# inhavl-shlee/AFI-GAN

Measured on AMD Instinct MI355X. Metric: stage1_G+D_step_images_per_s, higher is better.
Workload: dtype f32 via f16x3: two scaled fp16 pieces per operand, three f16 MFMAs per product, fp32 accumulate (tensors fp32)

## Files before the change

### afigan_amd/csrc/afi_common.h

```cpp
#pragma once
#include <hip/hip_runtime.h>
#include <stdint.h>
#include "../../include/afigan_hip.h"

typedef float f32x16 __attribute__((ext_vector_type(16)));
typedef float f32x4 __attribute__((ext_vector_type(4)));

#define AFI_LRELU_SLOPE 0.2f

#ifndef AFI_TRY
#define AFI_TRY(expr) do { int _s = (expr); if (_s != AFI_OK) return _s; } while (0)
#endif

struct AfiView {
    float* p;
    long long sN, sH, sW;
};

struct AfiBnLoad { const float* mean; const float* invstd; const float* gamma; const float* beta; };

struct AfiPixGemm {
    int N, H, W;
    int ntaps;
    int Ck;
// ... 38 lines not shown
#define AFI_WK6_STAGE_BYTES 6144
struct AfiWk6ImgJob { const float* B; long long b_sRow, b_sTap; int Ncols, Ck, ntaps, nKphase, b_rc; unsigned char* dst; };
struct AfiWk6Side { float* zero_p; long long zero_n4; const float* bl_dout; float* bl_dx; int bl_N, bl_H, bl_W, bl_C; };
struct AfiWk6ConvT { const float* W; unsigned char* dst; float* pack_dst; int Cin, Cout, mode, pad_; };

struct AfiWgradGemm {
    int N, H, W;
    int ntaps;
    int Mrows;
    int Ncols;
    AfiView DY; int dy_up; int CoutPhase;
    AfiView X;
    int x_stride, xH, xW;
    float* DW; long long dw_sRow, dw_sTap;
    long long dy_sTap, x_sTap;
    float alpha;
    int splitK;
};

#ifndef AFI_WINO4_POINTS
#define AFI_WINO4_POINTS 1
#endif
struct AfiF16Bound { const float* amax; int stride; int pad_; float cmul[36]; };

struct AfiColsumProb { const float* g; float* db; long long P, ld; int C; float alpha; };

static inline int afi_cdiv(long long a, long long b) { return (int)((a + b - 1) / b); }
```

### afigan_amd/csrc/afi_f16_split.h

```cpp
#pragma once
#include "afi_common.h"
typedef float f32x2 __attribute__((ext_vector_type(2)));
typedef unsigned int u32x2 __attribute__((ext_vector_type(2)));
typedef unsigned int u32x4 __attribute__((ext_vector_type(4)));
typedef _Float16 f16x8 __attribute__((ext_vector_type(8)));
typedef _Float16 f16x2 __attribute__((ext_vector_type(2)));


__device__ __forceinline__ float afi_f16_scale(float bound) {
    unsigned e = (__float_as_uint(bound) >> 23) & 0xffu;
    e = e < 27u ? 27u : e;
    return __uint_as_float((268u - e) << 23);
}
__device__ __forceinline__ float afi_pow2_inverse(float s) { return __uint_as_float((254u << 23) - __float_as_uint(s)); }

__device__ __forceinline__ void afi_split2_f16_pair(float x0, float x1, float s, unsigned& hi, unsigned& lo) {
    unsigned h, l;
    asm("v_fma_mixlo_f16 %0, %1, %2, 0" : "=v"(h) : "v"(x0), "v"(s));
    asm("v_fma_mixhi_f16 %0, %1, %2, 0" : "+v"(h) : "v"(x1), "v"(s));
    asm("v_fma_mixlo_f16 %0, %1, %2, -%3 op_sel:[0,0,0] op_sel_hi:[0,0,1]" : "=v"(l) : "v"(x0), "v"(s), "v"(h));
    asm("v_fma_mixhi_f16 %0, %1, %2, -%3 op_sel:[0,0,1] op_sel_hi:[0,0,1]" : "+v"(l) : "v"(x1), "v"(s), "v"(h));
    hi = h; lo = l;
}
__device__ __forceinline__ void afi_split2_f16_pair_cvt(float x0, float x1, float s, unsigned& hi, unsigned& lo) {
    const float a = x0 * s, b = x1 * s;
    const f16x2 h = __builtin_convertvector((f32x2){a, b}, f16x2);
    hi = __builtin_bit_cast(unsigned, h);
    const float r0 = a - (float)h[0], r1 = b - (float)h[1];
    lo = __builtin_bit_cast(unsigned, __builtin_convertvector((f32x2){r0, r1}, f16x2));
}
__device__ __forceinline__ void afi_split2_f16_x8_cvt(f32x4 v0, f32x4 v1, float s, u32x4& h, u32x4& l) {
    unsigned h0, h1, h2, h3, l0, l1, l2, l3;
    afi_split2_f16_pair_cvt(v0[0], v0[1], s, h0, l0);
    afi_split2_f16_pair_cvt(v0[2], v0[3], s, h1, l1);
    afi_split2_f16_pair_cvt(v1[0], v1[1], s, h2, l2);
    afi_split2_f16_pair_cvt(v1[2], v1[3], s, h3, l3);
    h = u32x4{h0, h1, h2, h3};
// ... 12 lines not shown
```

### afigan_amd/csrc/afi_launch.h

```cpp
#pragma once
#include "afi_common.h"

int afi_launch_pix_gemm(const AfiPixGemm& p, int b_rc, hipStream_t st);
int afi_launch_gemm_tn(const float* Q, const float* V, float* dU, int planes, long long rows_per_plane, int M, int N, hipStream_t st, bool deterministic = false);
int afi_launch_gemm_nt(const float* A, const float* B, float* C, int planes, long long rows_per_plane, int N, int K, hipStream_t st);
int afi_launch_split_bf16_tiles(const float* B, void* out, int planes, int N, int K, int split, hipStream_t st);
int afi_launch_gemm_nt_bf16_dma(const float* A, const void* Bsplit, float* C, int planes, long long rows_per_plane, int N, int K, int split, hipStream_t st);
int afi_launch_gemm_tn_bf16(const float* Q, const float* V, float* dU, int planes, long long rows_per_plane, int M, int N, int split, hipStream_t st, bool deterministic = false);
int afi_launch_split_f16_tiles(const float* B, void* out, int planes, int N, int K, hipStream_t st, int wkind = 0);
int afi_f16_image_begin(void* out, hipStream_t st);
float* afi_f16_image_wmax(void* out);
long long afi_f16_image_bytes(int planes, int N, int K);
int afi_launch_absmax_planes(const float* X, long long per_plane, int planes, float* out, hipStream_t st);
AfiF16Bound afi_f16_bound(const float* amax, int kind);
int afi_launch_gemm_nt_f16x3(const float* A, const void* Bimg, float* C, int planes, long long rows_per_plane, int N, int K, const AfiF16Bound& ab, hipStream_t st,
                             bool a_pre = false, long long nt256_min_tiles = 512, bool local_sums = false);
int afi_launch_gemm_tn_f16x3(const float* Q, const float* V, float* dU, int planes, long long rows_per_plane, int M, int N, const AfiF16Bound& qb, const AfiF16Bound& vb,
                             hipStream_t st, bool pre = false, bool deterministic = false);
int afi_launch_wgrad_gemm(const AfiWgradGemm& p, hipStream_t st);
int afi_launch_wgrad_gemm_group(const AfiWgradGemm* probs, int n, int wide, hipStream_t st);
int afi_launch_wgrad_gemm_group6(const AfiWgradGemm* probs, int n, hipStream_t st);
int afi_launch_pix_gemm_group(const AfiPixGemm* probs, int n, int b_rc, hipStream_t st);

long long afi_wk6_image_bytes(int Ncols, int Ck, int ntaps, int nKphase);
// ... 50 lines not shown
int afi_launch_maxpool3s2_same(AfiView x, int N, int H, int W, int C, float* out, hipStream_t st);
int afi_launch_fuse_swish(const float* a, const float* b, const float* c, const float* w, float* out, long long n, hipStream_t st);
int afi_launch_sgd(const void* descs_dev, int ntensors, long long max_n, float lr, float mom, float gscale, hipStream_t st);
int afi_launch_scale(float* p, long long n, float s, hipStream_t st);
int afi_launch_sum_accum(const float* v, long long n, float alpha, float* out, hipStream_t st);
int afi_launch_inc_i64(long long* p, hipStream_t st);
int afi_launch_invstd(const float* var, float* invstd, int C, hipStream_t st);

#ifndef AFI_STATS_MAX_ROWS
#define AFI_STATS_MAX_ROWS 1024
#endif
int afi_wino_stats_rows(long long T, int C);
int afi_launch_wino_weight(const float* w, float* U, int O, int I, int mode, hipStream_t st, float* wmax = nullptr);
int afi_launch_wino_input(AfiView x, int N, int H, int W, int C, long long Tpad, float* V, hipStream_t st, long long ldo = 0, float* amax = nullptr,
                          const AfiF16Bound* pre = nullptr);
int afi_launch_wino_output(const float* M, long long Tpad, int N, int H, int W, int C, const float* bias, float alpha, AfiView out, AfiView z,
                           hipStream_t st);
int afi_launch_wino_output_epi(const float* M, long long Tpad, const AfiPixGemm& p, hipStream_t st);
int afi_launch_wino_dy(AfiView dy, int N, int H, int W, int C, long long Tpad, float* Q, hipStream_t st, long long ldo = 0, float* amax = nullptr, const AfiF16Bound* pre = nullptr);
int afi_launch_wino_dw(const float* dU, float* dW, int O, int I, float alpha, hipStream_t st);
int afi_launch_wino4_input(AfiView x, int N, int H, int W, int C, long long Tpad, float* V, hipStream_t st, long long ldo = 0, float* amax = nullptr,
                           const AfiF16Bound* pre = nullptr);
int afi_launch_wino4_weight(const float* w, float* U, int O, int I, int mode, hipStream_t st, float* wmax = nullptr);
int afi_launch_wino4_output_epi(const float* M, long long Tpad, const AfiPixGemm& p, hipStream_t st);
int afi_launch_wino4_dy(AfiView dy, int N, int H, int W, int C, long long Tpad, float* Q, hipStream_t st, long long ldo = 0, float* amax = nullptr, const AfiF16Bound* pre = nullptr);
int afi_launch_wino4_dw(const float* dU, float* dW, int O, int I, float alpha, hipStream_t st);
```

### afigan_amd/csrc/nets.hip

```cpp
#include <string.h>
#include <stdlib.h>

#include "../../include/afigan_hip.h"
#include "afi_common.h"
#include "afi_launch.h"
#include <initializer_list>
#include <new>


#include <vector>
namespace {
struct SideStream {
    hipStream_t side = nullptr;
    std::vector<hipEvent_t> ring;
    size_t next = 0;
    bool init() {
        if (side) return true;
        if (hipStreamCreateWithFlags(&side, hipStreamNonBlocking) != hipSuccess) { side = nullptr; return false; }
        ring.resize(128);
        for (auto& e : ring)
            if (hipEventCreateWithFlags(&e, hipEventDisableTiming) != hipSuccess) return false;
        return true;
    }
    void destroy() {
// ... 181 lines not shown
static bool wino_eligible(const afi_ctx* cx, const AfiPixGemm& g, int b_rc) {
    if (!afi_opt(cx, AFI_OPT_WINOGRAD) || g.ntaps != 9 || g.gtap || g.r2_post) return false;
    const bool phases = g.nKphase == 4 && g.a_up == 2 && b_rc;
    if (!phases && (g.nKphase != 1 || g.a_up != 1)) return false;
    if (g.Ck < 128 || g.Ncols < 128 || (g.Ck & 3) || (g.Ncols & 3)) return false;
    if ((long long)g.N * g.H * g.W < wino_g_minpix(cx)) return false;
    const int I = b_rc ? g.Ncols : g.Ck;
    return g.b_sTap == I && g.b_sRow == 9LL * I && g.a_sgn == (b_rc ? -1 : 1);
}
static float* wino_wcache_slot(afi_ctx* cx, const float* w, int f4, int mode, int O, int I, long long need, bool& hit) {
    hit = false;
    if (!cx || !cx->wcache.buf) return nullptr;
    WinoWeightCache& c = cx->wcache;
    for (int i = 0; i < c.n; ++i) {
        const WinoWeightCache::Entry& e = c.e[i];
        if (e.w == w && e.f4 == f4 && e.mode == mode && e.O == O && e.I == I) { hit = true; return c.buf + e.off; }
    }
    if (c.n == 128 || c.used + need > c.floats) return nullptr;
    c.e[c.n++] = WinoWeightCache::Entry{w, f4, mode, O, I, c.used};
    float* slot = c.buf + c.used;
    c.used += need;
    return slot;
}

constexpr long long kWk6MaxPixels = 8192;
constexpr int kWk6MaxReq = 24;
struct Wk6Req { const float* key; const float* src; int Ncols, Ck, nKphase, b_rc; long long b_sRow, b_sTap; int convT; float* pack_dst; };
static inline Wk6Req wk6_req(const float* key, const float* src, int Ncols, int Ck, int nKphase, int b_rc, long long b_sRow, long long b_sTap) {
    return Wk6Req{key, src, Ncols, Ck, nKphase, b_rc, b_sRow, b_sTap, 0, nullptr};
}
static inline long long wk6_req_floats(int Ncols, int Ck, int nKphase) { return align4((afi_wk6_image_bytes(Ncols, Ck, 9, nKphase) + 3) / 4); }
struct Wk6Images {
    bool on = false;
    int n = 0;
    struct Ent { const float* key; const unsigned char* img; int nstages; } e[kWk6MaxReq];
    void attach(AfiPixGemm& g, const float* key, int c_lo = 0) const {
        if (!on || (c_lo & 31)) return;
        for (int i = 0; i < n; ++i)
            if (e[i].key == key) { g.Bimg = e[i].img; g.bimg_nstages = e[i].nstages; g.bimg_stage0 = (c_lo / 32) * g.ntaps; return; }
    }
};
static int wk6_build(afi_ctx* cx, Wk6Images& im, const Wk6Req* reqs, int n, float* arena, long long arena_floats, hipStream_t st,
                     const AfiWk6Side* side = nullptr, bool* side_done = nullptr, bool* ct_built = nullptr) {
    im.on = false; im.n = 0;
    if (side_done) *side_done = false;
    if (ct_built) *ct_built = false;
    if (n > kWk6MaxReq) return AFI_OK;
    struct CacheRollback {
        afi_ctx* cx; int n0; long long used0; bool keep = false;
        explicit CacheRollback(afi_ctx* c) : cx(c), n0(c ? c->wcache.n : 0), used0(c ? c->wcache.used : 0) {}
        ~CacheRollback() { if (cx && !keep) { cx->wcache.n = n0; cx->wcache.used = used0; } }
    } rollback(cx);
    AfiWk6ImgJob jobs[kWk6MaxReq];
    AfiWk6ConvT ct;
    bool have_ct = false;
    int nj = 0;
    long long used = 0;
    for (int i = 0; i < n; ++i) {
        const Wk6Req& r = reqs[i];
        const long long need = wk6_req_floats(r.Ncols, r.Ck, r.nKphase);
        bool hit = false;
        float* slot = wino_wcache_slot(cx, r.key,  4 + r.b_rc, r.nKphase, r.Ncols, r.Ck, need, hit);
        if (!slot) {
            if (!arena || used + need > arena_floats) { im.n = 0; return AFI_OK; }
            slot = arena + used; used += need; hit = false;
        }
        const int nst = afi_cdiv(r.Ck, 32) * 9 * r.nKphase;
        if (!hit && r.convT) {
            if (have_ct) { im.n = 0; return AFI_OK; }
            ct = AfiWk6ConvT{r.src, (unsigned char*)slot, r.pack_dst, r.convT == 1 ? r.Ck : r.Ncols, r.convT == 1 ? r.Ncols / 4 : r.Ck, r.convT == 1 ? 0 : 1, 0};
            have_ct = true;
        } else if (!hit) {
            jobs[nj++] = AfiWk6ImgJob{r.src, r.b_sRow, r.b_sTap, r.Ncols, r.Ck, 9, r.nKphase, r.b_rc, (unsigned char*)slot};
        }
        im.e[im.n++] = Wk6Images::Ent{r.key, (const unsigned char*)slot, nst};
// ... 3 lines not shown
        if (side && side_done) *side_done = true;
        if (have_ct && ct_built) *ct_built = true;
    }
    rollback.keep = true;
    im.on = true;
    return AFI_OK;
}
static inline bool wk6_shapes_ok(int C, int G, int R) { return (C % 32) == 0 && (G % 32) == 0 && 6 * R + 4 <= kWk6MaxReq; }
constexpr long long kWk6HiResMaxPixels = 4096;
static long long gen_wk6_fwd_floats(int C, int G, int R, long long P) {
    if (P > kWk6MaxPixels || !wk6_shapes_ok(C, G, R)) return 0;
    const int L = C + 4 * G;
    long long f = 3 * wk6_req_floats(C, C, 1) + wk6_req_floats(4 * C, C, 1);
    for (int k = 1; k <= 4; ++k) f += (long long)R * wk6_req_floats(G, C + (k - 1) * G, 1);
    return f + (long long)R * wk6_req_floats(C, L, 1);
}
static long long gen_wk6_bwd_floats(int C, int G, int R, long long P) {
    if (P > kWk6MaxPixels || !wk6_shapes_ok(C, G, R)) return 0;
    const int L = C + 4 * G;
    long long f = 3 * wk6_req_floats(C, C, 1) + wk6_req_floats(C, C, 4);
    for (int k = 1; k <= 4; ++k) f += (long long)R * wk6_req_floats(C + (k - 1) * G, G, 1);
    return f + (long long)R * wk6_req_floats(L, C, 1);
}

static int wino_run(afi_ctx* cx, const AfiPixGemm& g, const WinoForm& f, float* ws, long long ws_floats, float* part, long long part_floats, hipStream_t st) {
    AFI_TRY(afi_o16_refused(g));
    const int b_rc = f.kind == kWinoDgrad;
    const int nph = g.nKphase;
    const int K = g.Ck * nph, Nc = g.Ncols;
    if (ws_floats < wino_ws_floats(g.N, g.H, g.W, K, Nc)) return AFI_ERR_WORKSPACE;
    const int dtype = f.dtype, np = f.np; const long long Tpad = f.Tpad;
    const bool f4 = f.f4, dma = f.dma, f16 = f.f16;
    float* U = ws;
    float* Vb = U + align4((long long)np * K * Nc);
    float* Mb = Vb + align4(np * Tpad * K);
    float* Usp = Mb + align4(np * Tpad * Nc);
    float* amax = nullptr;
    bool have_u = false;
    if (g.no_wcache) {
    } else if (dma) {
        if (float* slot = wino_wcache_slot(cx, g.B, f4, b_rc | (dtype << 4), b_rc ? K : Nc, b_rc ? Nc : K, wino_usplit_floats(np, (long long)K * Nc), have_u)) Usp = slot;
    } else if (float* slot = wino_wcache_slot(cx, g.B, f4, b_rc, b_rc ? K : Nc, b_rc ? Nc : K, align4((long long)np * K * Nc), have_u)) U = slot;
    if (!have_u) {
        float* wmax = dma && f16 ? afi_f16_image_wmax(Usp) : nullptr;
        if (wmax) AFI_TRY(afi_f16_image_begin(Usp, st));
        AFI_TRY(f4 ? afi_launch_wino4_weight(g.B, U, b_rc ? K : Nc, b_rc ? Nc : K, b_rc, st, wmax)
                   : afi_launch_wino_weight(g.B, U, b_rc ? K : Nc, b_rc ? Nc : K, b_rc, st, wmax));
        if (dma) AFI_TRY(f16 ? afi_launch_split_f16_tiles(U, Usp, np, Nc, K, st, f4 ? 6 : 5) : afi_launch_split_bf16_tiles(U, Usp, np, Nc, K, dtype, st));
    }
    const bool a_pre = f.presplit && g.a_amax && g.a_amax_known;
    if (f16 && !(amax = g.a_amax ? g.a_amax : wino_amax_take(cx, ws, ws_floats, 1, st))) return AFI_ERR_LAUNCH;
    const AfiF16Bound abound = afi_f16_bound(amax, f4 ? 2 : 1);
    if (g.v_keep && !(f.keep && a_pre)) return AFI_ERR_BAD_ARG;
    if (g.v_keep) Vb = g.v_keep;
    for (int ph = 0; ph < nph; ++ph) {
        AfiView a = g.A;
        if (nph == 4) { a.p += (ph >> 1) * g.A.sH + (ph & 1) * g.A.sW; a.sH *= 2; a.sW *= 2; }
        float* raise = g.a_amax ? (g.a_amax_known ? nullptr : g.a_amax) : (f16 ? amax : nullptr);
        AFI_TRY(f4 ? afi_launch_wino4_input(a, g.N, g.H, g.W, g.Ck, Tpad, Vb + ph * g.Ck, st, K, raise, a_pre ? &abound : nullptr)
                   : afi_launch_wino_input(a, g.N, g.H, g.W, g.Ck, Tpad, Vb + ph * g.Ck, st, K, raise, a_pre ? &abound : nullptr));
    }
    if (dma) {
        if (f16) AFI_TRY(afi_launch_gemm_nt_f16x3(Vb, Usp, Mb, np, Tpad, Nc, K, abound, st, a_pre, afi_opt(cx, AFI_OPT_F16_NT256_MIN_TILES), g.nt_local_sums != 0));
        else AFI_TRY(afi_launch_gemm_nt_bf16_dma(Vb, Usp, Mb, np, Tpad, Nc, K, dtype, st));
        return f4 ? afi_launch_wino4_output_epi(Mb, Tpad, g, st) : afi_launch_wino_output_epi(Mb, Tpad, g, st);
    }
// ... 774 lines not shown
    float* wp = ws + l.o_wp;
    AfiView x = V(xv);
    auto buf = [&](int r) { return dense_view(ws + l.o_buf + (long long)r * l.P * L, H, W, L); };
    AfiView t = dense_view(ws + l.o_t, H, W, C), a7 = dense_view(ws + l.o_a7, H, W, C);
    AfiView u = dense_view(ws + l.o_u, 2 * H, 2 * W, C);

    Wk6Images im;
    bool packed = false;
    if (p.fwd.six) {
        Wk6Req rq[kWk6MaxReq];
        AFI_TRY(wk6_build(cx, im, rq, gen_fwd_image_reqs(p, prm, wp, rq), ws + l.o_img, l.n_img, st, nullptr, nullptr, &packed));
    }
    if (!packed) {
        bool hit = false;
        const long long wp_floats = 36LL * C * C;
        if (float* slot = wino_wcache_slot(cx, prm->wT,  2, 0, C, C, align4(wp_floats), hit)) {
            if (!hit) AFI_TRY(afi_launch_convT_pack(prm->wT, slot, C, C, st));
            if (hipMemcpyAsync(wp, slot, sizeof(float) * wp_floats, hipMemcpyDeviceToDevice, st) != hipSuccess) return AFI_ERR_LAUNCH;
        } else {
            AFI_TRY(afi_launch_convT_pack(prm->wT, wp, C, C, st));
        }
    }
    {
        AfiPixGemm g = conv_fwd_desc(x, N, H, W, C, prm->w0, prm->b0, C, buf(0));
        g.lrelu = 1;
        im.attach(g, prm->w0);
        AFI_TRY(PG(g, 0));
    }
    for (int r = 0; r < R; ++r) {
        AfiView b = buf(r);
        const bool last = (r == R - 1);
        auto conv5_desc = [&](int c_lo, int nch) {
            AfiPixGemm g = conv_fwd_desc(ch_off(b, c_lo), N, H, W, nch, prm->rdb_w[r][4] + c_lo, nullptr, C, last ? t : buf(r + 1));
            g.b_sRow = 9LL * L; g.b_sTap = L;
            g.alpha = last ? rs * rs : rs;
            if (c_lo == 0) {
                g.R1 = b; g.r1_lo = 0; g.r1_hi = C; g.r1s = last ? rs : 1.f;
                if (last) { g.R2 = buf(0); g.r2s = 1.f; g.r2_lo = 0; g.r2_hi = C; }
            } else {
                g.beta = 1.f;
            }
            im.attach(g, prm->rdb_w[r][4], c_lo);
            return g;
        };
        if (p.fwd.batched) {
            for (int j = 0; j <= 4; ++j) {
// ... 217 lines not shown
    AfiView x = V(xv);
    AfiView t = dense_view(ws + l.o_t, H, W, C), a7 = dense_view(ws + l.o_a7, H, W, C);
    AfiView u = dense_view(ws + l.o_u, 2 * H, 2 * W, C);
    AfiView dOut = dense_view(dout, 2 * H, 2 * W, C);
    AfiView dU = dense_view(scratch + s.o_du, 2 * H, 2 * W, C);
    AfiView gA = dense_view(scratch + s.o_ga, H, W, C), gB = dense_view(scratch + s.o_gb, H, W, C);
    float* dwp = scratch + s.o_dwp;
    const bool one_fill = p.bwd.one_fill && gr->wT;
    const long long n_dwp = align4(36LL * C * C), n_fill = (one_fill ? n_dwp : 0) + (long long)R * s.n_rdbw;
    float* const fill = scratch + s.o_rdbw - (one_fill ? n_dwp : 0);
    bool filled = false, skip_grad_done = false;
    if (p.bwd.images) {
        Wk6Req rq[kWk6MaxReq];
        AfiWk6Side side;
        memset(&side, 0, sizeof(side));
        if (one_fill && (((uintptr_t)fill) & 15) == 0) { side.zero_p = fill; side.zero_n4 = n_fill / 4; }
        if (dx && (C & 3) == 0) { side.bl_dout = dout; side.bl_dx = dx; side.bl_N = N; side.bl_H = H; side.bl_W = W; side.bl_C = C; }
        bool rode = false;
        AFI_TRY(wk6_build(cx, c.im, rq, gen_bwd_image_reqs(p, prm, dx != nullptr, rq), scratch + s.o_img, s.n_img, st, &side, &rode));
        filled = rode && side.zero_p;
        skip_grad_done = rode && side.bl_dx;
    }
    if (p.bwd.pack_growth && !filled && hipMemsetAsync(fill, 0, sizeof(float) * (size_t)n_fill, st) != hipSuccess) return AFI_ERR_LAUNCH;

    if (gr->w9) AFI_TRY(c.wgrad(dOut, u, 2 * H, 2 * W, C, C, gr->w9, 1.f));
    if (gr->b9) AFI_TRY(c.colsum(dout, 4 * P, C, C, gr->b9));
    {
        AfiPixGemm g = conv_dgrad_desc(dOut, N, 2 * H, 2 * W, C, prm->w9, C, dU);
        g.Z = u; g.z_lo = 0; g.z_hi = C;
        c.im.attach(g, prm->w9);
        AFI_TRY(c.PG(g, 1));
    }
    c.fk.after_main();
    if (gr->wT) {
        hipStream_t sd = c.fk.side;
        if (!one_fill && hipMemsetAsync(dwp, 0, sizeof(float) * 36LL * C * C, sd) != hipSuccess) return AFI_ERR_LAUNCH;
        if (p.bwd.grouped) {
            AFI_TRY(c.df.defer(cx, convT_wgrad_desc(dU, a7, N, H, W, C, C, dwp, 1.f), st));
            c.df.convT = true;
        } else if (gen_wino_wgrad_ok(cx, p, 4 * C, C, P)) {
            WinoWgradOpt o;
            o.dy_phases = 4; o.accumulate = false;
            AFI_TRY(wino_wgrad(cx, dU, a7, N, H, W, 4 * C, C, dwp, 1.f, scratch + s.o_wino2, s.n_wino, sd, o));
        } else {
            AFI_TRY(wgrad_launch(cx, convT_wgrad_desc(dU, a7, N, H, W, C, C, dwp, 1.f), sd));
        }
// ... 166 lines not shown

static int disc_fwd(afi_ctx_t* ctx, const afi_disc_params_t* prm, afi_view_t xv, int N, int H, int W, int halves, float* logits, int training, float* ws,
                    long long ws_floats, void* stream) {
    afi_ctx* cx = ctx; (void)cx;
    AFI_CTX_CHECK(ctx);
    AFI_TRY(disc_check(prm));
    const bool stats_only = training == 3;
    if (N <= 0 || H <= 0 || W <= 0 || !ws || !xv.p || (!logits && !stats_only)) return AFI_ERR_BAD_ARG;
    if ((halves != 1 && halves != 2) || N % halves) return AFI_ERR_BAD_ARG;
    const DiscPlan pl = disc_plan(cx, prm->F, N, H, W, training, halves);
    const DiscWs& l = pl.ws;
    if (ws_floats < l.total) return AFI_ERR_WORKSPACE;
    hipStream_t st = (hipStream_t)stream;
    float* const part_ = ws + l.o_part;
    const long long part_n_ = l.n_part;
    auto PG = [&](AfiPixGemm g, int b_rc) { g.partial = part_; g.partial_floats = part_n_; return afi_launch_pix_gemm(g, b_rc, st); };
    const long long P = l.P;
    float* red = ws + l.o_red;
    AfiView in = V(xv);
    const bool wino = pl.wino, tail = pl.tail;
    const long long Ph = P / halves;
    float* amax = ws + l.o_amax;
    if (pl.fwd_amax && hipMemsetAsync(amax, 0, 16 * sizeof(float), st) != hipSuccess) return AFI_ERR_LAUNCH;
    bool in_known = false;
    if (pl.x_amax) {
        AFI_TRY(afi_launch_view_absmax(in, N, H, W, prm->F[0], amax, st));
        in_known = true;
    }
    for (int n = 0; n < 3; ++n) {
        const int ci = prm->F[n], co = prm->F[n + 1];
        float* c = ws + l.o_c[n]; float* y = ws + l.o_y[n];
        float* mean = ws + l.o_mean[n]; float* invstd = ws + l.o_invstd[n];
        const DiscPlan::Block& b = pl.b[n];
        int stats_rows = 0;
        double* stats = (double*)(ws + l.o_stats);
        const bool fuse_stats = b.stats && (((uintptr_t)stats) & 7) == 0;
        if (wino) {
            if (b.keep && !in_known) return AFI_ERR_LAUNCH;
            WinoConvOpt o;
            if (fuse_stats) { o.stats = stats; o.stats_rows = &stats_rows; }
            o.in_amax = pl.fwd_amax ? amax + 4 * n : nullptr; o.in_amax_known = in_known;
            o.v_keep = b.keep ? ws + l.o_vkeep[n] : nullptr; o.local_sums = b.local_sums;
            AFI_TRY(wino_conv(cx, b.fwd.kind, in, N, H, W, ci, prm->w[n], co, prm->b[n], dense_view(c, H, W, co), null_view(), ws + l.o_wino, l.n_wino, part_,
                              part_n_, st, o));
        } else {
            AFI_TRY(PG(conv_fwd_desc(in, N, H, W, ci, prm->w[n], prm->b[n], co, dense_view(c, H, W, co)), 0));
// ... 45 lines not shown
    }
    return AFI_OK;
}

static int disc_bwd(afi_ctx_t* ctx, const afi_disc_params_t* prm, const afi_disc_params_t* gr, afi_view_t xv, int N, int H, int W, int halves, const float* ws,
                    const float* dlogits, float* dx, float* scratch, long long scratch_floats, void* stream) {
    afi_ctx* cx = ctx; (void)cx;
    AFI_CTX_CHECK(ctx);
    AFI_TRY(disc_check(prm));
    if (!gr || N <= 0 || H <= 0 || W <= 0 || !ws || !dlogits || !scratch) return AFI_ERR_BAD_ARG;
    if ((halves != 1 && halves != 2) || N % halves) return AFI_ERR_BAD_ARG;
    const DiscPlan pl = disc_plan(cx, prm->F, N, H, W, 1, halves);
    const DiscWs& l = pl.ws;
    const DiscBwdWs& s = pl.bws;
    if (scratch_floats < s.total) return AFI_ERR_WORKSPACE;
    hipStream_t st = (hipStream_t)stream;
    float* const part_ = scratch + s.o_part;
    const long long part_n_ = s.n_part;
    auto PG = [&](AfiPixGemm g, int b_rc) { g.partial = part_; g.partial_floats = part_n_; return afi_launch_pix_gemm(g, b_rc, st); };
    const long long P = l.P;
    float* red = scratch + s.o_red;
    float* red2 = scratch + s.o_red2;
    float* dd9 = scratch + s.o_dd9;
    Fork fk(cx, st, P <= kSideStreamMaxPixels);
    hipStream_t sd = fk.side;
    const bool wino = pl.wino, tail = pl.tail;
    const int F3 = prm->F[3];
    float* gmax = scratch + s.o_amax;
    const bool bwd_amax = pl.bwd_amax;
    if (bwd_amax && hipMemsetAsync(gmax, 0, 16 * sizeof(float), st) != hipSuccess) return AFI_ERR_LAUNCH;
    const float* xmax = ws + l.o_amax;
    if (gr->b3) AFI_TRY(afi_launch_sum_accum(dlogits, P, 1.f, gr->b3, sd));
    AFI_TRY(afi_launch_stencil9_scatter(dlogits, dd9, 16, N, H, W, st));
    fk.after_main();
    AfiView y2 = dense_view(ws + l.o_y[2], H, W, F3);
    if (gr->w3 && !tail) {
        AfiWgradGemm g = conv_wgrad_desc(dense_view(dd9, H, W, 16), y2, N, H, W, 9, F3, gr->w3, 1.f);
        g.ntaps = 1; g.dw_sRow = F3; g.dw_sTap = 0;
        AFI_TRY(wgrad_launch(cx, g, sd));
    }
    if (!tail) {
        AfiPixGemm g = pix_default(N, H, W);
        g.ntaps = 1; g.a_sgn = -1; g.Ck = 9; g.Ncols = F3; g.CoutPhase = F3;
        g.A = dense_view(dd9, H, W, 16); g.B = prm->w3; g.b_sRow = F3; g.b_sTap = 0;
        g.O = dense_view(scratch + s.o_g[2], H, W, F3);
        AFI_TRY(PG(g, 1));
// ... 62 lines not shown
```

### afigan_amd/csrc/winograd.hip

```cpp
#include "afi_common.h"
#include "afi_launch.h"
#include "afi_epilogue.h"
#include "afi_f16_split.h"

__device__ __forceinline__ float afi_amax4(float m, f32x4 v) {
    return fmaxf(fmaxf(m, fmaxf(fabsf(v[0]), fabsf(v[1]))), fmaxf(fabsf(v[2]), fabsf(v[3])));
}
__device__ __forceinline__ void afi_amax_publish(float m, float* slot) {
    __shared__ float red[16];
#pragma unroll
    for (int o = 32; o > 0; o >>= 1) m = fmaxf(m, __shfl_xor(m, o));
    const int tid = threadIdx.x + blockDim.x * threadIdx.y, nw = (blockDim.x * blockDim.y + 63) >> 6;
    if ((tid & 63) == 0) red[tid >> 6] = m;
    __syncthreads();
    if (tid == 0) {
        for (int w = 1; w < nw; ++w) m = fmaxf(m, red[w]);
        const unsigned bits = __float_as_uint(m);
        if (bits > __hip_atomic_load((const unsigned*)slot, __ATOMIC_RELAXED, __HIP_MEMORY_SCOPE_AGENT)) (void)atomicMax((unsigned*)slot, bits);
    }
}

__device__ __forceinline__ void afi_store_split4(float* dst_row, int c, f32x4 v, float s) {
    unsigned char* b = (unsigned char*)dst_row + (c >> 5) * 128 + (c & 31) * 2;
    unsigned h0, h1, l0, l1;
    afi_split2_f16_pair_cvt(v[0], v[1], s, h0, l0);
    afi_split2_f16_pair_cvt(v[2], v[3], s, h1, l1);
    *(u32x2*)b = u32x2{h0, h1};
    *(u32x2*)(b + 64) = u32x2{l0, l1};
}

static bool afi_epilogue_is_simple_host(const AfiPixGemm& p) {
    return p.o_up == 1 && p.beta == 0.f && !p.R1.p && !p.R2.p && !p.r2_post && p.oH >= p.H && p.oW >= p.W &&
           (!p.Z.p || (p.z_lo == 0 && p.z_hi >= p.Ncols));
}
static unsigned wino_grid(long long work_items) {
    long long g = (work_items + 255) / 256;
    if (g > 8192) g = 8192;
    if (g < 1) g = 1;
    return (unsigned)g;
}

__global__ void afi_wino_weight_kernel(const float* __restrict__ w, float* __restrict__ U, int O, int I, int mode, float* wmax) {
    const long long total = (long long)O * I;
    float am = 0.f;
    for (long long e = (long long)blockIdx.x * blockDim.x + threadIdx.x; e < total; e += (long long)gridDim.x * blockDim.x) {
        const int i = (int)(e % I), o = (int)(e / I);
        float g[3][3];
#pragma unroll
        for (int t = 0; t < 9; ++t) {
            const int tt = mode ? 8 - t : t;
            g[t / 3][t % 3] = w[((long long)o * 9 + tt) * I + i];
            am = fmaxf(am, fabsf(g[t / 3][t % 3]));
        }
        float a[4][3];
#pragma unroll
        for (int j = 0; j < 3; ++j) {
            a[0][j] = g[0][j];
            a[1][j] = 0.5f * (g[0][j] + g[1][j] + g[2][j]);
            a[2][j] = 0.5f * (g[0][j] - g[1][j] + g[2][j]);
            a[3][j] = g[2][j];
        }
        const long long plane = (long long)O * I;
        const long long off = mode ? (long long)i * O + o : (long long)o * I + i;
#pragma unroll
        for (int r = 0; r < 4; ++r) {
            const float u0 = a[r][0], u1 = 0.5f * (a[r][0] + a[r][1] + a[r][2]), u2 = 0.5f * (a[r][0] - a[r][1] + a[r][2]), u3 = a[r][2];
            U[(4 * r + 0) * plane + off] = u0;
            U[(4 * r + 1) * plane + off] = u1;
            U[(4 * r + 2) * plane + off] = u2;
            U[(4 * r + 3) * plane + off] = u3;
        }
    }
    if (wmax) afi_amax_publish(am, wmax);
}
int afi_launch_wino_weight(const float* w, float* U, int O, int I, int mode, hipStream_t st, float* wmax) {
    if (O <= 0 || I <= 0) return AFI_ERR_BAD_ARG;
    hipLaunchKernelGGL(afi_wino_weight_kernel, dim3(wino_grid((long long)O * I)), dim3(256), 0, st, w, U, O, I, mode, wmax);
    return hipGetLastError() == hipSuccess ? AFI_OK : AFI_ERR_LAUNCH;
}

template <int AM = 0>
__global__ __launch_bounds__(256) void afi_wino_input_kernel(const AfiView x, int N, int H, int W, int C, int Th, int Tw, long long T,
                                                             long long Tpad, float* __restrict__ Vout, long long ldo, float* amax, const AfiF16Bound bnd) {
    constexpr bool AMAX = AM == 1;
    const float src_max = AM == 2 ? bnd.amax[0] : 0.f;
    const int C4 = C >> 2;
    const long long total = Tpad * C4;
    const long long plane = Tpad * ldo;
    float am = 0.f;
    for (long long e = (long long)blockIdx.x * blockDim.x + threadIdx.x; e < total; e += (long long)gridDim.x * blockDim.x) {
        const int c = (int)(e % C4) * 4;
        const long long t = e / C4;
        float* dst = Vout + t * ldo + c;
// ... 468 lines not shown
        float u[6];
        wino4_g3(a[r][0], a[r][1], a[r][2], u);
        if (!mode) {
#pragma unroll
            for (int c = 0; c < 6; ++c)
                if (ok) U[(6 * r + c) * plane + (long long)o * I + i] = u[c];
            continue;
        }
#pragma unroll
        for (int c = 0; c < 6; ++c) {
            __syncthreads();
            tile[to][ti] = u[c];
            __syncthreads();
            if (ok2) U[(6 * r + c) * plane + (long long)oi * O + oo] = tile[ti][to];
        }
    }
}
int afi_launch_wino4_weight(const float* w, float* U, int O, int I, int mode, hipStream_t st, float* wmax) {
    if (O <= 0 || I <= 0) return AFI_ERR_BAD_ARG;
    hipLaunchKernelGGL(afi_wino4_weight_kernel, dim3((I + 31) / 32, (O + 31) / 32), dim3(32, 32), 0, st, w, U, O, I, mode, wmax);
    return hipGetLastError() == hipSuccess ? AFI_OK : AFI_ERR_LAUNCH;
}

template <bool SIMPLE, bool STATS = false>
__global__ __launch_bounds__(256) void afi_wino4_output_epi_kernel(const float* __restrict__ Min, long long Tpad, int Th, int Tw, long long T,
                                                                   const AfiPixGemm p) {
    const int C = p.Ncols, C4 = C >> 2;
    const long long total = T * C4;
    const long long plane = Tpad * C;
    f64x4w st0 = {0, 0, 0, 0}, st1 = {0, 0, 0, 0};
    for (long long e = (long long)blockIdx.x * blockDim.x + threadIdx.x; e < total; e += (long long)gridDim.x * blockDim.x) {
        const int c = (int)(e % C4) * 4;
        const long long t = e / C4;
        const int tx = (int)(t % Tw); const long long r = t / Tw; const int ty = (int)(r % Th); const int n = (int)(r / Th);
        const float* src = Min + t * C + c;
        f32x4 s[4][6];
#pragma unroll
        for (int j = 0; j < 6; ++j) {
            const f32x4 m0 = __builtin_nontemporal_load((const f32x4*)(src + (0 * 6 + j) * plane)), m1 = __builtin_nontemporal_load((const f32x4*)(src + (1 * 6 + j) * plane));
            const f32x4 m2 = __builtin_nontemporal_load((const f32x4*)(src + (2 * 6 + j) * plane)), m3 = __builtin_nontemporal_load((const f32x4*)(src + (3 * 6 + j) * plane));
            const f32x4 m4 = __builtin_nontemporal_load((const f32x4*)(src + (4 * 6 + j) * plane)), m5 = __builtin_nontemporal_load((const f32x4*)(src + (5 * 6 + j) * plane));
            wino4_at(m0, m1, m2, m3, m4, m5, s[0][j], s[1][j], s[2][j], s[3][j]);
        }
#pragma unroll
        for (int i = 0; i < 4; ++i) {
            const int yy = 4 * ty + i;
// ... 135 lines not shown
```

Baseline: 28.69.

## Build Winograd f16 weight images directly in batched multi-job kernels

Adds a batched path that turns raw 3x3 conv weights straight into the split-f16 swizzled tile images used by the Winograd DMA GEMM. A per-job absmax kernel runs first, then a single build kernel does the transform and the hi/lo split. This replaces the per-layer sequence of Winograd weight transform, fp32 U buffer, and separate split/pack launches. Forward and backward passes for the generator and discriminator now pre-build all uncached weight images in one or two launches at stage start. The cost is extra LDS transpose work for the dgrad mode and a new wcache rollback wrapper that has to stay consistent with slot allocation.

```diff
diff --git a/afigan_amd/csrc/afi_common.h b/afigan_amd/csrc/afi_common.h
--- a/afigan_amd/csrc/afi_common.h
+++ b/afigan_amd/csrc/afi_common.h
@@ -84,6 +84,7 @@
 #define AFI_WINO4_POINTS 1
 #endif
 struct AfiF16Bound { const float* amax; int stride; int pad_; float cmul[36]; };
+struct AfiWinoImgJob { const float* w; unsigned char* dst; int O, I, f4, mode; };
 
 struct AfiColsumProb { const float* g; float* db; long long P, ld; int C; float alpha; };
 
diff --git a/afigan_amd/csrc/afi_f16_split.h b/afigan_amd/csrc/afi_f16_split.h
--- a/afigan_amd/csrc/afi_f16_split.h
+++ b/afigan_amd/csrc/afi_f16_split.h
@@ -13,6 +13,7 @@
     return __uint_as_float((268u - e) << 23);
 }
 __device__ __forceinline__ float afi_pow2_inverse(float s) { return __uint_as_float((254u << 23) - __float_as_uint(s)); }
+__device__ __forceinline__ int afi_f16_tile_chunk_off(int row, int ch) { return row * 64 + (((ch ^ (-(row >> 2))) & 3) << 4); }
 
 __device__ __forceinline__ void afi_split2_f16_pair(float x0, float x1, float s, unsigned& hi, unsigned& lo) {
     unsigned h, l;
diff --git a/afigan_amd/csrc/afi_launch.h b/afigan_amd/csrc/afi_launch.h
--- a/afigan_amd/csrc/afi_launch.h
+++ b/afigan_amd/csrc/afi_launch.h
@@ -96,6 +96,7 @@
 int afi_launch_wino4_input(AfiView x, int N, int H, int W, int C, long long Tpad, float* V, hipStream_t st, long long ldo = 0, float* amax = nullptr,
                            const AfiF16Bound* pre = nullptr);
 int afi_launch_wino4_weight(const float* w, float* U, int O, int I, int mode, hipStream_t st, float* wmax = nullptr);
+int afi_launch_wino_weight_images(const AfiWinoImgJob* jobs, int n, float* wmax_slots, hipStream_t st);
 int afi_launch_wino4_output_epi(const float* M, long long Tpad, const AfiPixGemm& p, hipStream_t st);
 int afi_launch_wino4_dy(AfiView dy, int N, int H, int W, int C, long long Tpad, float* Q, hipStream_t st, long long ldo = 0, float* amax = nullptr, const AfiF16Bound* pre = nullptr);
 int afi_launch_wino4_dw(const float* dU, float* dW, int O, int I, float alpha, hipStream_t st);
diff --git a/afigan_amd/csrc/nets.hip b/afigan_amd/csrc/nets.hip
--- a/afigan_amd/csrc/nets.hip
+++ b/afigan_amd/csrc/nets.hip
@@ -227,6 +227,11 @@
     c.used += need;
     return slot;
 }
+struct CacheRollback {
+    afi_ctx* cx; int n0; long long used0; bool keep = false;
+    explicit CacheRollback(afi_ctx* c) : cx(c), n0(c ? c->wcache.n : 0), used0(c ? c->wcache.used : 0) {}
+    ~CacheRollback() { if (cx && !keep) { cx->wcache.n = n0; cx->wcache.used = used0; } }
+};
 
 constexpr long long kWk6MaxPixels = 8192;
 constexpr int kWk6MaxReq = 24;
@@ -251,11 +256,7 @@
     if (side_done) *side_done = false;
     if (ct_built) *ct_built = false;
     if (n > kWk6MaxReq) return AFI_OK;
-    struct CacheRollback {
-        afi_ctx* cx; int n0; long long used0; bool keep = false;
-        explicit CacheRollback(afi_ctx* c) : cx(c), n0(c ? c->wcache.n : 0), used0(c ? c->wcache.used : 0) {}
-        ~CacheRollback() { if (cx && !keep) { cx->wcache.n = n0; cx->wcache.used = used0; } }
-    } rollback(cx);
+    CacheRollback rollback(cx);
     AfiWk6ImgJob jobs[kWk6MaxReq];
     AfiWk6ConvT ct;
     bool have_ct = false;
@@ -305,6 +306,32 @@
     for (int k = 1; k <= 4; ++k) f += (long long)R * wk6_req_floats(C + (k - 1) * G, G, 1);
     return f + (long long)R * wk6_req_floats(L, C, 1);
 }
+
+static inline bool wino_direct_build(const afi_ctx* cx) { return !(afi_opt(cx, AFI_OPT_F16_PRESPLIT) & 2); }
+static inline bool wino_direct_image(const afi_ctx* cx, const WinoForm& f) { return f.dma && f.f16 && wino_direct_build(cx); }
+struct WinoImgBatch {
+    afi_ctx* cx; CacheRollback rollback; bool open;
+    AfiWinoImgJob jobs[24];
+    int nj = 0;
+    explicit WinoImgBatch(afi_ctx* c) : cx(c), rollback(c), open(c && c->wcache.buf && wino_direct_build(c)) {}
+    void add(const float* w, int K, int Nc, const WinoForm& f) {
+        if (!open) return;
+        if (!wino_direct_image(cx, f) || nj == 24) { open = false; return; }
+        const int b_rc = f.kind == kWinoDgrad;
+        bool hit = false;
+        float* slot = wino_wcache_slot(cx, w, f.f4, b_rc | (f.dtype << 4), b_rc ? K : Nc, b_rc ? Nc : K, wino_usplit_floats(f.np, (long long)K * Nc), hit);
+        if (slot && !hit) jobs[nj++] = AfiWinoImgJob{w, (unsigned char*)slot, b_rc ? K : Nc, b_rc ? Nc : K, f.f4 ? 1 : 0, b_rc};
+    }
+    void add(const AfiPixGemm& g, int b_rc, long long n_wino, bool fwd_f4) {
+        if (!open || g.Bimg || g.no_wcache || n_wino <= 0 || !wino_eligible(cx, g, b_rc)) return;
+        add(g.B, g.Ck * g.nKphase, g.Ncols, wino_form(cx, g, b_rc, fwd_f4));
+    }
+    int build(float* wmax_slots, hipStream_t st) {
+        if (cx) AFI_TRY(afi_launch_wino_weight_images(jobs, nj, wmax_slots, st));
+        rollback.keep = true;
+        return AFI_OK;
+    }
+};
 
 static int wino_run(afi_ctx* cx, const AfiPixGemm& g, const WinoForm& f, float* ws, long long ws_floats, float* part, long long part_floats, hipStream_t st) {
     AFI_TRY(afi_o16_refused(g));
@@ -324,7 +351,10 @@
     } else if (dma) {
         if (float* slot = wino_wcache_slot(cx, g.B, f4, b_rc | (dtype << 4), b_rc ? K : Nc, b_rc ? Nc : K, wino_usplit_floats(np, (long long)K * Nc), have_u)) Usp = slot;
     } else if (float* slot = wino_wcache_slot(cx, g.B, f4, b_rc, b_rc ? K : Nc, b_rc ? Nc : K, align4((long long)np * K * Nc), have_u)) U = slot;
-    if (!have_u) {
+    if (!have_u && wino_direct_image(cx, f)) {
+        const AfiWinoImgJob job{g.B, (unsigned char*)Usp, b_rc ? K : Nc, b_rc ? Nc : K, f4 ? 1 : 0, b_rc};
+        AFI_TRY(afi_launch_wino_weight_images(&job, 1, U, st));
+    } else if (!have_u) {
         float* wmax = dma && f16 ? afi_f16_image_wmax(Usp) : nullptr;
         if (wmax) AFI_TRY(afi_f16_image_begin(Usp, st));
         AFI_TRY(f4 ? afi_launch_wino4_weight(g.B, U, b_rc ? K : Nc, b_rc ? Nc : K, b_rc, st, wmax)
@@ -1145,6 +1175,28 @@
         }
     }
     {
+        WinoImgBatch ib(cx);
+        auto want = [&](AfiPixGemm g, const float* key, int c_lo = 0) { if (key) im.attach(g, key, c_lo); ib.add(g, 0, l.n_wino, p.fwd.f4); };
+        want(conv_fwd_desc(x, N, H, W, C, prm->w0, prm->b0, C, buf(0)), prm->w0);
+        for (int r = 0; r < R && !p.fwd.batched && ib.open; ++r) {
+            if (p.fwd.xbatch) {
+                const float* const wk[4] = {prm->rdb_w[r][0], prm->rdb_w[r][1], prm->rdb_w[r][2], prm->rdb_w[r][3]};
+                bool hit = false;
+                if (float* slot = wino_wcache_slot(cx, prm->rdb_w[r][0],  3, 0, 4 * G, C, l.n_rdbx, hit)) {
+                    if (!hit) AFI_TRY(afi_launch_rdb_xpart_pack(wk, slot, C, G, st));
+                    want(conv_fwd_desc(buf(r), N, H, W, C, slot, nullptr, 4 * G, ch_off(buf(r), C)), nullptr);
+                }
+            } else {
+                for (int k = 1; k <= 4; ++k) want(conv_fwd_desc(buf(r), N, H, W, C + (k - 1) * G, prm->rdb_w[r][k - 1], nullptr, G, buf(r)), nullptr);
+            }
+            want(conv_fwd_desc(buf(r), N, H, W, L, prm->rdb_w[r][4], nullptr, C, buf(r)), prm->rdb_w[r][4]);
+        }
+        want(conv_fwd_desc(t, N, H, W, C, prm->w7, prm->b7, C, a7), prm->w7);
+        want(convT_fwd_desc(a7, N, H, W, C, wp, prm->bT, C, u), prm->wT);
+        want(conv_fwd_desc(u, N, 2 * H, 2 * W, C, prm->w9, prm->b9, C, V(outv)), prm->w9);
+        AFI_TRY(ib.build(ws + l.o_wino, st));
+    }
+    {
         AfiPixGemm g = conv_fwd_desc(x, N, H, W, C, prm->w0, prm->b0, C, buf(0));
         g.lrelu = 1;
         im.attach(g, prm->w0);
@@ -1408,6 +1460,29 @@
         skip_grad_done = rode && side.bl_dx;
     }
     if (p.bwd.pack_growth && !filled && hipMemsetAsync(fill, 0, sizeof(float) * (size_t)n_fill, st) != hipSuccess) return AFI_ERR_LAUNCH;
+    {
+        WinoImgBatch ib(cx);
+        const int G = prm->G;
+        auto want = [&](AfiPixGemm g, const float* key) { if (key) c.im.attach(g, key); ib.add(g, 1, s.n_wino, false); };
+        want(conv_dgrad_desc(dOut, N, 2 * H, 2 * W, C, prm->w9, C, dU), prm->w9);
+        want(convT_dgrad_desc(dU, N, H, W, C, ws + l.o_wp, C, gA), prm->wT);
+        want(conv_dgrad_desc(gA, N, H, W, C, prm->w7, C, gB), prm->w7);
+        for (int r = R - 1; r >= 0 && ib.open; --r) {
+            want(conv_dgrad_desc(gB, N, H, W, C, prm->rdb_w[r][4], L, c.dbuf(r)), prm->rdb_w[r][4]);
+            if (p.bwd.batch_growth) {
+                const float* const wk[4] = {prm->rdb_w[r][0], prm->rdb_w[r][1], prm->rdb_w[r][2], prm->rdb_w[r][3]};
+                bool hit = false;
+                if (float* slot = wino_wcache_slot(cx, prm->rdb_w[r][0],  3, 0, 4 * G, C, s.n_rdbx, hit)) {
+                    if (!hit) AFI_TRY(afi_launch_rdb_xpart_pack(wk, slot, C, G, st));
+                    want(conv_dgrad_desc(c.dbuf(r), N, H, W, 4 * G, slot, C, c.dbuf(r)), nullptr);
+                }
+            } else {
+                for (int k = 4; k >= 1; --k) want(conv_dgrad_desc(c.dbuf(r), N, H, W, G, prm->rdb_w[r][k - 1], C + (k - 1) * G, c.dbuf(r)), prm->rdb_w[r][k - 1]);
+            }
+        }
+        if (dx) want(conv_dgrad_desc(gB, N, H, W, C, prm->w0, C, dense_view(dx, H, W, C)), prm->w0);
+        AFI_TRY(ib.build(scratch + s.o_wino, st));
+    }
 
     if (gr->w9) AFI_TRY(c.wgrad(dOut, u, 2 * H, 2 * W, C, C, gr->w9, 1.f));
     if (gr->b9) AFI_TRY(c.colsum(dout, 4 * P, C, C, gr->b9));
@@ -1620,6 +1695,11 @@
     const long long Ph = P / halves;
     float* amax = ws + l.o_amax;
     if (pl.fwd_amax && hipMemsetAsync(amax, 0, 16 * sizeof(float), st) != hipSuccess) return AFI_ERR_LAUNCH;
+    if (wino) {
+        WinoImgBatch ib(cx);
+        for (int n = 0; n < 3; ++n) ib.add(prm->w[n], prm->F[n], prm->F[n + 1], pl.b[n].fwd);
+        AFI_TRY(ib.build(ws + l.o_wino, st));
+    }
     bool in_known = false;
     if (pl.x_amax) {
         AFI_TRY(afi_launch_view_absmax(in, N, H, W, prm->F[0], amax, st));
@@ -1711,6 +1791,11 @@
     float* red = scratch + s.o_red;
     float* red2 = scratch + s.o_red2;
     float* dd9 = scratch + s.o_dd9;
+    if (pl.wino) {
+        WinoImgBatch ib(cx);
+        for (int n = 2; n >= (dx ? 0 : 1); --n) ib.add(prm->w[n], prm->F[n + 1], prm->F[n], wino_form(cx, N, H, W, prm->F[n + 1], prm->F[n], kWinoDgrad));
+        AFI_TRY(ib.build(scratch + s.o_wino, st));
+    }
     Fork fk(cx, st, P <= kSideStreamMaxPixels);
     hipStream_t sd = fk.side;
     const bool wino = pl.wino, tail = pl.tail;
diff --git a/afigan_amd/csrc/winograd.hip b/afigan_amd/csrc/winograd.hip
--- a/afigan_amd/csrc/winograd.hip
+++ b/afigan_amd/csrc/winograd.hip
@@ -1,3 +1,6 @@
+#include <stdint.h>
+#include <string.h>
+
 #include "afi_common.h"
 #include "afi_launch.h"
 #include "afi_epilogue.h"
@@ -40,6 +43,13 @@
     return (unsigned)g;
 }
 
+template <typename T>
+__device__ __forceinline__ void wino2_g3(const T g0, const T g1, const T g2, T (&a)[4]) {
+    a[0] = g0;
+    a[1] = 0.5f * (g0 + g1 + g2);
+    a[2] = 0.5f * (g0 - g1 + g2);
+    a[3] = g2;
+}
 __global__ void afi_wino_weight_kernel(const float* __restrict__ w, float* __restrict__ U, int O, int I, int mode, float* wmax) {
     const long long total = (long long)O * I;
     float am = 0.f;
@@ -55,20 +65,19 @@
         float a[4][3];
 #pragma unroll
         for (int j = 0; j < 3; ++j) {
-            a[0][j] = g[0][j];
-            a[1][j] = 0.5f * (g[0][j] + g[1][j] + g[2][j]);
-            a[2][j] = 0.5f * (g[0][j] - g[1][j] + g[2][j]);
-            a[3][j] = g[2][j];
+            float col[4];
+            wino2_g3(g[0][j], g[1][j], g[2][j], col);
+#pragma unroll
+            for (int r = 0; r < 4; ++r) a[r][j] = col[r];
         }
         const long long plane = (long long)O * I;
         const long long off = mode ? (long long)i * O + o : (long long)o * I + i;
 #pragma unroll
         for (int r = 0; r < 4; ++r) {
-            const float u0 = a[r][0], u1 = 0.5f * (a[r][0] + a[r][1] + a[r][2]), u2 = 0.5f * (a[r][0] - a[r][1] + a[r][2]), u3 = a[r][2];
-            U[(4 * r + 0) * plane + off] = u0;
-            U[(4 * r + 1) * plane + off] = u1;
-            U[(4 * r + 2) * plane + off] = u2;
-            U[(4 * r + 3) * plane + off] = u3;
+            float u[4];
+            wino2_g3(a[r][0], a[r][1], a[r][2], u);
+#pragma unroll
+            for (int c = 0; c < 4; ++c) U[(4 * r + c) * plane + off] = u[c];
         }
     }
     if (wmax) afi_amax_publish(am, wmax);
@@ -583,6 +592,165 @@
     return hipGetLastError() == hipSuccess ? AFI_OK : AFI_ERR_LAUNCH;
 }
 
+#define AFI_WINO_IMG_MAXJOBS 64
+#define AFI_WINO_IMG_MAX_FLOATS 8192
+struct AfiWinoImgTable {
+    int njobs, pad_;
+    int unit_start[AFI_WINO_IMG_MAXJOBS + 1];
+    int max_start[AFI_WINO_IMG_MAXJOBS + 1];
+    float cmul2[16], cmul4[36];
+    float* wmax;
+    AfiWinoImgJob j[AFI_WINO_IMG_MAXJOBS];
+};
+__global__ __launch_bounds__(256) void afi_wino_img_max_kernel(const AfiWinoImgTable tb) {
+    const int b = (int)blockIdx.x;
+    int ji = 0;
+    while (ji + 1 < tb.njobs && b >= tb.max_start[ji + 1]) ++ji;
+    const AfiWinoImgJob& jb = tb.j[ji];
+    const long long n4 = (long long)jb.O * 9 * jb.I / 4;
+    const long long i0 = (long long)(b - tb.max_start[ji]) * (AFI_WINO_IMG_MAX_FLOATS / 4) + threadIdx.x;
+    constexpr int NL = AFI_WINO_IMG_MAX_FLOATS / 1024;
+    float m = 0.f;
+    if (i0 + (NL - 1) * 256 < n4) {
+        f32x4 v[NL];
+#pragma unroll
+        for (int k = 0; k < NL; ++k) v[k] = *(const f32x4*)(jb.w + 4 * (i0 + k * 256));
+#pragma unroll
+        for (int k = 0; k < NL; ++k) m = afi_amax4(m, v[k]);
+    } else {
+#pragma unroll
+        for (int k = 0; k < NL; ++k) {
+            const long long i = i0 + k * 256;
+            if (i < n4) m = afi_amax4(m, *(const f32x4*)(jb.w + 4 * i));
+        }
+    }
+    afi_amax_publish(m, tb.wmax + ji);
+}
+template <bool F4>
+__device__ __forceinline__ void afi_wino_img_unit(const AfiWinoImgJob& jb, int unit, float wmax, const float* __restrict__ cmul, float* lds) {
+    constexpr int NP1 = F4 ? 6 : 4;
+    constexpr int LD = 65, PL = 32 * LD;
+    const int tid = threadIdx.x, mode = jb.mode;
+    const int I = jb.I, N = mode ? jb.I : jb.O, K = mode ? jb.O : jb.I;
+    const int nkc = K >> 5;
+    const int slab = unit / nkc, kc = unit - slab * nkc;
+    float g[9][8];
+    if (!mode) {
+        const float* src = jb.w + (long long)(slab * 64 + (tid >> 2)) * 9 * I + kc * 32 + 8 * (tid & 3);
+#pragma unroll
+        for (int t = 0; t < 9; ++t) {
+            const f32x4 v0 = *(const f32x4*)(src + (long long)t * I), v1 = *(const f32x4*)(src + (long long)t * I + 4);
+#pragma unroll
+            for (int e = 0; e < 4; ++e) { g[t][e] = v0[e]; g[t][4 + e] = v1[e]; }
+        }
+    } else {
+        const float* src = jb.w + (long long)(kc * 32 + (tid >> 3)) * 9 * I + slab * 64 + 4 * (tid & 7);
+#pragma unroll
+        for (int t = 0; t < 9; ++t) {
+            const f32x4 v0 = *(const f32x4*)(src + (long long)(8 - t) * I), v1 = *(const f32x4*)(src + (long long)(8 - t) * I + 32);
+#pragma unroll
+            for (int e = 0; e < 4; ++e) { g[t][e] = v0[e]; g[t][4 + e] = v1[e]; }
+        }
+    }
+    const int srow = tid >> 2, sch = tid & 3;
+    const int row = (slab & 1) * 64 + srow;
+    unsigned char* img = jb.dst + 512 + (((long long)(slab >> 1)) * nkc + kc) * 16384LL + afi_f16_tile_chunk_off(row, sch);
+    const long long plane_bytes = (long long)(N >> 7) * nkc * 16384LL;
+#pragma unroll
+    for (int r = 0; r < NP1; ++r) {
+        float u[NP1][8];
+#pragma unroll
+        for (int e = 0; e < 8; ++e) {
+            float a[3];
+#pragma unroll
+            for (int j = 0; j < 3; ++j) {
+                float col[NP1];
+                if constexpr (F4) wino4_g3(g[j][e], g[3 + j][e], g[6 + j][e], col); else wino2_g3(g[j][e], g[3 + j][e], g[6 + j][e], col);
+                a[j] = col[r];
+            }
+            float uu[NP1];
+            if constexpr (F4) wino4_g3(a[0], a[1], a[2], uu); else wino2_g3(a[0], a[1], a[2], uu);
+#pragma unroll
+            for (int c = 0; c < NP1; ++c) u[c][e] = uu[c];
+        }
+        if (mode) {
+            __syncthreads();
+            float* wr = lds + (tid >> 3) * LD + 4 * (tid & 7);
+#pragma unroll
+            for (int c = 0; c < NP1; ++c)
+#pragma unroll
+                for (int e = 0; e < 4; ++e) { wr[c * PL + e] = u[c][e]; wr[c * PL + 32 + e] = u[c][4 + e]; }
+            __syncthreads();
+            const float* rd = lds + (8 * sch) * LD + srow;
+#pragma unroll
+            for (int c = 0; c < NP1; ++c)
+#pragma unroll
+                for (int e = 0; e < 8; ++e) u[c][e] = rd[c * PL + e * LD];
+        }
+#pragma unroll
+        for (int c = 0; c < NP1; ++c) {
+            const int plane = NP1 * r + c;
+            const float s = afi_f16_scale(wmax * cmul[plane]);
+            unsigned h0, h1, h2, h3, l0, l1, l2, l3;
+            afi_split2_f16_pair(u[c][0], u[c][1], s, h0, l0);
+            afi_split2_f16_pair(u[c][2], u[c][3], s, h1, l1);
+            afi_split2_f16_pair(u[c][4], u[c][5], s, h2, l2);
+            afi_split2_f16_pair(u[c][6], u[c][7], s, h3, l3);
+            unsigned char* d = img + plane * plane_bytes;
+            *(u32x4*)d = u32x4{h0, h1, h2, h3};
+            *(u32x4*)(d + 8192) = u32x4{l0, l1, l2, l3};
+        }
+    }
+}
+__global__ __launch_bounds__(256) void afi_wino_img_build_kernel(const AfiWinoImgTable tb) {
+    __shared__ float lds[6 * 32 * 65];
+    const int b = (int)blockIdx.x;
+    int ji = 0;
+    while (ji + 1 < tb.njobs && b >= tb.unit_start[ji + 1]) ++ji;
+    const AfiWinoImgJob& jb = tb.j[ji];
+    const int unit = b - tb.unit_start[ji];
+    const float wmax = tb.wmax[ji];
+    const float* cmul = jb.f4 ? tb.cmul4 : tb.cmul2;
+    if (unit == 0 && threadIdx.x < 128) {
+        const int t = threadIdx.x, np = jb.f4 ? 36 : 16;
+        ((float*)jb.dst)[t] = t < np ? afi_f16_scale(wmax * cmul[t]) : (t == 64 ? wmax : 0.f);
+    }
+    if (jb.f4) afi_wino_img_unit<true>(jb, unit, wmax, cmul, lds);
+    else afi_wino_img_unit<false>(jb, unit, wmax, cmul, lds);
+}
+int afi_launch_wino_weight_images(const AfiWinoImgJob* jobs, int n, float* wmax_slots, hipStream_t st) {
+    if (n <= 0) return AFI_OK;
+    if (!jobs || !wmax_slots) return AFI_ERR_BAD_ARG;
+    const size_t nfill = ((size_t)n + AFI_WINO_IMG_MAXJOBS - 1) / AFI_WINO_IMG_MAXJOBS * AFI_WINO_IMG_MAXJOBS;
+    if (hipMemsetAsync(wmax_slots, 0, sizeof(float) * nfill, st) != hipSuccess) return AFI_ERR_LAUNCH;
+    const AfiF16Bound b2 = afi_f16_bound(nullptr, 5), b4 = afi_f16_bound(nullptr, 6);
+    for (int done = 0; done < n; done += AFI_WINO_IMG_MAXJOBS) {
+        const int cnt = n - done < AFI_WINO_IMG_MAXJOBS ? n - done : AFI_WINO_IMG_MAXJOBS;
+        AfiWinoImgTable tb;
+        tb.njobs = cnt; tb.pad_ = 0;
+        tb.wmax = wmax_slots + done;
+        memcpy(tb.cmul2, b2.cmul, sizeof(tb.cmul2));
+        memcpy(tb.cmul4, b4.cmul, sizeof(tb.cmul4));
+        long long units = 0, mblocks = 0;
+        for (int i = 0; i < cnt; ++i) {
+            const AfiWinoImgJob& j = jobs[done + i];
+            if (!j.w || !j.dst || j.O <= 0 || j.I <= 0 || (j.mode != 0 && j.mode != 1)) return AFI_ERR_BAD_ARG;
+            const int N = j.mode ? j.I : j.O, K = j.mode ? j.O : j.I;
+            if ((N % 128) || (K % 32) || (j.I & 3) || (((uintptr_t)j.w | (uintptr_t)j.dst) & 15)) return AFI_ERR_UNSUPPORTED;
+            tb.j[i] = j;
+            tb.unit_start[i] = (int)units; tb.max_start[i] = (int)mblocks;
+            units += (long long)(N / 64) * (K / 32);
+            mblocks += ((long long)j.O * 9 * j.I + AFI_WINO_IMG_MAX_FLOATS - 1) / AFI_WINO_IMG_MAX_FLOATS;
+            if (units > 0x3fffffffLL || mblocks > 0x3fffffffLL) return AFI_ERR_UNSUPPORTED;
+        }
+        for (int i = cnt; i <= AFI_WINO_IMG_MAXJOBS; ++i) { tb.unit_start[i] = (int)units; tb.max_start[i] = (int)mblocks; }
+        for (int i = cnt; i < AFI_WINO_IMG_MAXJOBS; ++i) tb.j[i] = AfiWinoImgJob{nullptr, nullptr, 0, 0, 0, 0};
+        hipLaunchKernelGGL(afi_wino_img_max_kernel, dim3((unsigned)mblocks), dim3(256), 0, st, tb);
+        hipLaunchKernelGGL(afi_wino_img_build_kernel, dim3((unsigned)units), dim3(256), 0, st, tb);
+    }
+    return hipGetLastError() == hipSuccess ? AFI_OK : AFI_ERR_LAUNCH;
+}
+
 template <bool SIMPLE, bool STATS = false>
 __global__ __launch_bounds__(256) void afi_wino4_output_epi_kernel(const float* __restrict__ Min, long long Tpad, int Th, int Tw, long long T,
                                                                    const AfiPixGemm p) {
```

New measurement: 29.14 (median of 6 runs). 1.02x the previous value.
